# quantumgizmos/bp_osd

Hardware: AMD Instinct MI355X
Metric: syndromes decoded/sec (whole node) + logical error rate, HGP [[1922,50]] p=0.05 (higher is better)
Workload: dtype f64; 1 GPU; h1922_ms_cs7: [[1922,50]] HGP (31x31 circulant 1+x^2+x^5) hz 961x1922, min-sum BP variable scaling, max_iter=1922, osd_cs order 7, iid bit-flip q=0.05; per_gpu_batch=131072, global_batch=131072, bp_variant=0, pipelined_steps=2, hw_queues=4, batches=2 distinct seeded batches alternate over the timed steps

## Files before the change

### bp_osd_amd/_lib.py

```python
from __future__ import annotations

import ctypes as C
import os

_HERE = os.path.dirname(os.path.abspath(__file__))
LIB_PATH = os.environ.get("BPOSD_LIB") or os.path.join(_HERE, "libbposd_mi355x.so")

BPOSD_OK = 0
BPOSD_ERR_INVALID = -1
BPOSD_ERR_UNSUPPORTED = -2
BPOSD_ERR_HIP = -3
BPOSD_ERR_NO_DEVICE = -4

EXPORTED_SYMBOLS = (
    "bposd_device_count",
    "bposd_version",
    "bposd_create",
    "bposd_update_channel_probs",
    "bposd_decode_batch",
    "bposd_decode_batch_packed",
    "bposd_decode_batch_async",
    "bposd_decode_batch_packed_async",
    "bposd_decode_batch_device",
    "bposd_decode_batch_device_packed",
    "bposd_decode_batch_select",
    "bposd_decode_batch_select_device",
    "bposd_pack_rows_device",
    "bposd_pack_rows_device_lane",
    "bposd_synchronize",
    "bposd_num_lanes",
    "bposd_last_lane",
    "bposd_synchronize_lane",
    "bposd_lane_timing",
    "bposd_host_alloc",
    "bposd_host_free",
    "bposd_last_timing",
    "bposd_info",
    "bposd_posterior_llr",
    "bposd_set_bp_variant",
    "bposd_set_osd_variant",
    "bposd_last_osd_kernel",
    "bposd_mc_create",
    "bposd_mc_run",
    "bposd_mc_fetch",
    "bposd_mc_device_bytes",
    "bposd_mc_last_error",
    "bposd_mc_destroy",
    "bposd_last_error",
    "bposd_destroy",
)

DEBUG_SYMBOLS = (
    "bposd_layout_info",
    "bposd_bp_kernel_info",
    "bposd_debug_local_layout",
    "bposd_debug_class_layout",
    "bposd_debug_last_instance",
)


class BposdConfig(C.Structure):
    _fields_ = [
        ("device", C.c_int32),
        ("bp_method", C.c_int32),
        ("ms_scaling_factor", C.c_double),
        ("max_iter", C.c_int32),
        ("osd_method", C.c_int32),
        ("osd_order", C.c_int32),
        ("sort_tie_policy", C.c_int32),
        ("weight_fn", C.c_int32),
        ("schedule", C.c_int32),
        ("ps_clip", C.c_double),
        ("osd_e_bit_order", C.c_int32),
        ("ps_math_form", C.c_int32),
    ]


class BposdMcConfig(C.Structure):
    _fields_ = [
        ("device", C.c_int32),
        ("channel_update", C.c_int32),
        ("seed", C.c_uint64),
        ("capacity", C.c_int64),
    ]


MC_UPDATE = {None: 0, "x->z": 1, "z->x": 2}
MC_ITEMS = {"error_x": 0, "error_z": 1, "syndrome_x": 2, "syndrome_z": 3, "flags": 4, "syndrome_x_packed": 5, "syndrome_z_packed": 6}


_lib = None


def load():
    global _lib
    if _lib is not None:
        return _lib
    if not os.path.exists(LIB_PATH):
        raise RuntimeError(
            f"{LIB_PATH} not found: build it with `python -c 'import __graft_entry__ as g; g.build()'` "
            "(hipcc --offload-arch=gfx950).  bp_osd_amd has no CPU fallback."
        )
    os.environ.setdefault("GPU_MAX_HW_QUEUES", "8")
    lib = C.CDLL(LIB_PATH)
    vp = C.c_void_p
    lib.bposd_device_count.restype = C.c_int
    lib.bposd_version.restype = C.c_char_p
    lib.bposd_create.argtypes = [C.POINTER(BposdConfig), vp, vp, C.c_int32, C.c_int32, vp, C.POINTER(vp)]
    lib.bposd_create.restype = C.c_int
    lib.bposd_update_channel_probs.argtypes = [vp, vp]
    lib.bposd_update_channel_probs.restype = C.c_int
    lib.bposd_decode_batch.argtypes = [vp, vp, C.c_int64, vp, vp, vp, vp, vp, vp]
    lib.bposd_decode_batch.restype = C.c_int
    lib.bposd_decode_batch_packed.argtypes = [vp, vp, C.c_int64, vp, vp, vp, vp, vp]
    lib.bposd_decode_batch_packed.restype = C.c_int
    lib.bposd_decode_batch_async.argtypes = [vp, vp, C.c_int64, vp, vp, vp, vp, vp, vp]
    lib.bposd_decode_batch_async.restype = C.c_int
    lib.bposd_decode_batch_packed_async.argtypes = [vp, vp, C.c_int64, vp, vp, vp, vp, vp]
    lib.bposd_decode_batch_packed_async.restype = C.c_int
    lib.bposd_decode_batch_device.argtypes = [vp, vp, C.c_int64, vp, vp, vp, vp, vp, vp]
    lib.bposd_decode_batch_device.restype = C.c_int
    lib.bposd_decode_batch_device_packed.argtypes = [vp, vp, C.c_int64, vp, vp, vp, vp, vp]
    lib.bposd_decode_batch_device_packed.restype = C.c_int
    lib.bposd_decode_batch_select.argtypes = [vp, vp, C.c_int64, vp, vp, vp, vp, vp, vp, vp, vp]
    lib.bposd_decode_batch_select.restype = C.c_int
    lib.bposd_decode_batch_select_device.argtypes = [vp, vp, C.c_int64, vp, vp, vp, vp, vp, vp, vp, vp]
    lib.bposd_decode_batch_select_device.restype = C.c_int
    lib.bposd_pack_rows_device.argtypes = [vp, vp, C.c_int64, C.c_int32, vp]
    lib.bposd_pack_rows_device.restype = C.c_int
    lib.bposd_synchronize.argtypes = [vp]
    lib.bposd_synchronize.restype = C.c_int
    lib.bposd_num_lanes.argtypes = [vp]
    lib.bposd_num_lanes.restype = C.c_int
    lib.bposd_last_lane.argtypes = [vp]
    lib.bposd_last_lane.restype = C.c_int
    lib.bposd_synchronize_lane.argtypes = [vp, C.c_int32]
    lib.bposd_synchronize_lane.restype = C.c_int
    lib.bposd_lane_timing.argtypes = [vp, C.c_int32, C.POINTER(C.c_double), C.POINTER(C.c_double),
                                      C.POINTER(C.c_int64), C.POINTER(C.c_int64)]
    lib.bposd_lane_timing.restype = C.c_int
    lib.bposd_host_alloc.argtypes = [C.c_size_t]
    lib.bposd_host_alloc.restype = vp
    lib.bposd_host_free.argtypes = [vp]
    lib.bposd_host_free.restype = None
    lib.bposd_last_timing.argtypes = [vp, C.POINTER(C.c_double), C.POINTER(C.c_double),
                                      C.POINTER(C.c_int64), C.POINTER(C.c_int64)]
    lib.bposd_last_timing.restype = C.c_int
    lib.bposd_info.argtypes = [vp, C.POINTER(C.c_int32), C.POINTER(C.c_int32), C.POINTER(C.c_int32),
                               C.POINTER(C.c_int32)]
    lib.bposd_info.restype = C.c_int
    lib.bposd_layout_info.argtypes = [vp, C.POINTER(C.c_int64), C.POINTER(C.c_int64), C.POINTER(C.c_int64)]
    lib.bposd_layout_info.restype = C.c_int
    lib.bposd_pack_rows_device_lane.argtypes = [vp, C.c_int32, vp, C.c_int64, C.c_int32, vp]
    lib.bposd_pack_rows_device_lane.restype = C.c_int
    lib.bposd_posterior_llr.argtypes = [vp, vp, C.c_int64, vp, vp, vp, vp]
    lib.bposd_posterior_llr.restype = C.c_int
    lib.bposd_bp_kernel_info.argtypes = [vp, C.POINTER(C.c_int32), vp]
    lib.bposd_bp_kernel_info.restype = C.c_int
    lib.bposd_debug_local_layout.argtypes = [vp, vp, C.c_int32, C.c_int32, vp]
    lib.bposd_debug_local_layout.restype = C.c_int
    lib.bposd_debug_class_layout.argtypes = [vp, vp, C.c_int32, C.c_int32, vp, vp, vp, vp, vp, vp]
    lib.bposd_debug_class_layout.restype = C.c_int
    lib.bposd_debug_last_instance.argtypes = [vp, vp, vp]
    lib.bposd_debug_last_instance.restype = C.c_int
    lib.bposd_set_osd_variant.argtypes = [vp, C.c_int32]
    lib.bposd_set_osd_variant.restype = C.c_int
    lib.bposd_last_osd_kernel.argtypes = [vp]
    lib.bposd_last_osd_kernel.restype = C.c_int
    lib.bposd_set_bp_variant.argtypes = [vp, C.c_int32]
    lib.bposd_set_bp_variant.restype = C.c_int
    lib.bposd_last_error.argtypes = [vp]
    lib.bposd_last_error.restype = C.c_char_p
    lib.bposd_destroy.argtypes = [vp]
    lib.bposd_destroy.restype = None
    lib.bposd_mc_create.argtypes = [C.POINTER(BposdMcConfig), vp, vp, vp, vp, C.c_int32, vp, vp, C.c_int32, C.c_int32, vp, vp, C.c_int32,
                                    vp, vp, vp, vp, C.POINTER(vp)]
    lib.bposd_mc_create.restype = C.c_int
    lib.bposd_mc_run.argtypes = [vp, C.c_uint64, C.c_int64, C.POINTER(C.c_int64)]
    lib.bposd_mc_run.restype = C.c_int
    lib.bposd_mc_fetch.argtypes = [vp, C.c_int32, vp, C.c_size_t]
    lib.bposd_mc_fetch.restype = C.c_int
    lib.bposd_mc_device_bytes.argtypes = [vp]
    lib.bposd_mc_device_bytes.restype = C.c_int64
    lib.bposd_mc_last_error.argtypes = [vp]
    lib.bposd_mc_last_error.restype = C.c_char_p
    lib.bposd_mc_destroy.argtypes = [vp]
    lib.bposd_mc_destroy.restype = None
    _lib = lib
    return lib


def check_mc(lib, mc, rc):
    if rc == BPOSD_OK:
        return
    msg = lib.bposd_mc_last_error(mc)
    msg = msg.decode() if msg else f"error {rc}"
    if rc in (BPOSD_ERR_INVALID, BPOSD_ERR_UNSUPPORTED):
        raise ValueError(msg)
    raise RuntimeError(msg)


def check(lib, handle, rc):
    if rc == BPOSD_OK:
        return
    msg = lib.bposd_last_error(handle)
    msg = msg.decode() if msg else f"error {rc}"
    if rc in (BPOSD_ERR_INVALID, BPOSD_ERR_UNSUPPORTED):
        raise ValueError(msg)
    raise RuntimeError(msg)
```

### bp_osd_amd/csrc/bp_local_kernel.hip.h

```cpp
#pragma once
#include <hip/hip_runtime.h>
#include <stdint.h>

#include "bp_kernel.hip.h"

#ifndef BPOSD_BPL_SIGN_ON_MAG
#define BPOSD_BPL_SIGN_ON_MAG 0
#endif
namespace bposd {

struct BpLocalParams {
    int m, n;
    long long B;
    int max_iter;
    double ms_scaling;
    int osd_enabled;
    int mp;
    const uint8_t* __restrict__ synd;
    const double* __restrict__ llr0;
    const uint8_t* __restrict__ sel;
    const double* __restrict__ llr0_alt;
    const int* __restrict__ pos_chk;
    const int* __restrict__ pos_bit;
    const int* __restrict__ pos_alo;
    const int* __restrict__ pos_ahi;
    const int* __restrict__ pos_dl;
    const int* __restrict__ grp_dl;
    uint8_t* __restrict__ out_bp;
    uint8_t* __restrict__ out_osd0;
    uint8_t* __restrict__ out_osdw;
    uint8_t* __restrict__ out_conv;
    int* __restrict__ out_iters;
    double* __restrict__ out_llr;
    double* __restrict__ llr_ws;
    double* __restrict__ llr_tmp;
    int* __restrict__ osd_list;
    int* __restrict__ counters;
    unsigned long long* __restrict__ iter_total;
    int* __restrict__ tail_flag;
    int packed_io;
};

__host__ __device__ inline size_t bp_local_lds_bytes(int mp) {
    return ((size_t)4 * mp + 2) * 8 + (size_t)(mp / 32 + 2) * 4 + 8 * 4;
}

template <int DL>
__device__ __forceinline__ void bit_update(double l0, double R, double X, double Y, double& llr, double& oR, double& oX,
                                           double& oY) {
    const double c0 = DL == 0 ? R : (DL == 1 ? Y : X);
    const double c1 = DL == 0 ? X : (DL == 1 ? R : Y);
    const double c2 = DL == 0 ? Y : (DL == 1 ? X : R);
    const double pre0 = l0;
    const double pre1 = pre0 + c0;
    const double pre2 = pre1 + c1;
    llr = pre2 + c2;
    const double o2 = pre2;
    const double o1 = pre1 + c2;
    const double o0 = pre0 + (c2 + c1);
    oR = DL == 0 ? o0 : (DL == 1 ? o1 : o2);
    oX = DL == 0 ? o1 : (DL == 1 ? o2 : o0);
    oY = DL == 0 ? o2 : (DL == 1 ? o0 : o1);
}

__device__ __forceinline__ void bit_update_mixed(int dlv, double l0, double R, double X, double Y, double& llr, double& oR,
                                                 double& oX, double& oY) {
    const bool d0 = dlv == 0, d1 = dlv == 1;
    const double c0 = d0 ? R : (d1 ? Y : X);
    const double c1 = d0 ? X : (d1 ? R : Y);
    const double c2 = d0 ? Y : (d1 ? X : R);
    const double pre0 = l0;
    const double pre1 = pre0 + c0;
    const double pre2 = pre1 + c1;
    llr = pre2 + c2;
    const double o2 = pre2;
    const double o1 = pre1 + c2;
    const double o0 = pre0 + (c2 + c1);
    oR = d0 ? o0 : (d1 ? o1 : o2);
    oX = d0 ? o1 : (d1 ? o2 : o0);
    oY = d0 ? o2 : (d1 ? o0 : o1);
}

__device__ __forceinline__ int bpl_table_load(const int* base, unsigned int lane_off, unsigned int const_off) {
    asm volatile("" : "+v"(lane_off));
    return *(const int*)((const char*)base + (lane_off + const_off));
}

static_assert(__is_trivially_copyable(BpLocalParams) && alignof(BpLocalParams) <= 8, "BpLocalParams is copied into the kernarg segment as it is");
typedef const __attribute__((address_space(4))) BpLocalParams* bpl_args_ptr;
__device__ __forceinline__ bpl_args_ptr bpl_args() {
    bpl_args_ptr a = (bpl_args_ptr)__builtin_amdgcn_kernarg_segment_ptr();
    asm volatile("" : "+s"(a));
    return a;
}

template <int CPT, int MPT, int MINW, bool EARLY, bool UPRIOR, bool PACKED = false>
__global__ __launch_bounds__(MPT / CPT, MINW) void bp_local_kernel(const BpLocalParams P) {
    extern __shared__ __attribute__((aligned(16))) unsigned char smem[];
    const int m = P.m, n = P.n;
#ifdef BPOSD_DEBUG
    if (blockIdx.x == 0 && threadIdx.x == 0 && (bpl_args()->m != P.m || bpl_args()->counters != P.counters)) __builtin_trap();
#endif
    constexpr int NT = MPT / CPT;
    constexpr int MP = MPT;
    const int tid = threadIdx.x;
    const int lane = tid & 63;
    const int wave = __builtin_amdgcn_readfirstlane(tid >> 6);
    constexpr int NB = 2 * CPT;

    double* msg_plain = reinterpret_cast<double*>(smem);
    msg_ptr msg = (msg_ptr)msg_plain;
    unsigned int* diffw = reinterpret_cast<unsigned int*>(msg_plain + (size_t)4 * MP + 2);
    int* sh = reinterpret_cast<int*>(diffw + (MP / 32 + 2));
    const unsigned int diffw_base = (unsigned int)(uintptr_t)(__attribute__((address_space(3))) unsigned char*)diffw;

    typedef __attribute__((address_space(3))) unsigned char* lds_bytes;
    const unsigned int msg_base = (unsigned int)(uintptr_t)(lds_bytes)smem;
    unsigned int alo[NB], ahi[NB];
    int dl[NB];
    unsigned int dlpack = 0u;
    double l0[UPRIOR ? 1 : NB];
    if (UPRIOR) {
        const double v = bpl_args()->llr0[0];
        l0[0] = __hiloint2double(__builtin_amdgcn_readfirstlane(__double2hiint(v)), __builtin_amdgcn_readfirstlane(__double2loint(v)));
    }
#define BPL_L0(r) l0[UPRIOR ? 0 : (r)]
#define BPL_AT(a) ((msg_ptr)(uintptr_t)(a))
#define BPL_BIT(r) bpl_table_load(bpl_args()->pos_bit, (unsigned int)tid * 4u, (unsigned int)((((r) & 1) * MP + ((r) >> 1) * NT) * 4))
#pragma unroll
    for (int j = 0; j < CPT; ++j) {
        const int p = tid + j * NT;
#pragma unroll
        for (int b = 0; b < 2; ++b) {
            const int r = 2 * j + b;
            if (!UPRIOR) {
                const int bit = BPL_BIT(r);
                l0[r] = bit >= 0 ? bpl_args()->llr0[bit] : 1.0;
            }
            alo[r] = msg_base + 8u * (unsigned int)bpl_args()->pos_alo[b * MP + p];
            ahi[r] = msg_base + 8u * (unsigned int)bpl_args()->pos_ahi[b * MP + p];
            dl[r] = __builtin_amdgcn_readfirstlane(bpl_args()->grp_dl[b * (MP >> 6) + (p >> 6)]);
            dlpack |= (unsigned int)bpl_args()->pos_dl[b * MP + p] << (2 * r);
        }
    }

    const int want_llr_s = __builtin_amdgcn_readfirstlane(bpl_args()->out_llr != nullptr ? 1 : 0);
    auto want_llr = [&]() -> bool {
        int w = want_llr_s;
        asm volatile("" : "+s"(w));
        return w != 0;
    };
    for (;;) {
        if (tid == 0) {
            int zero = 0;
            asm volatile("" : "+v"(zero));
            sh[0] = zero;
            sh[1] = zero;
            sh[2] = atomicAdd(&bpl_args()->counters[0], 1);
        }
        __syncthreads();
        const long long s = __builtin_amdgcn_readfirstlane(sh[2]);
        if (s >= P.B) {
            if (s == P.B && tid == 0 && bpl_args()->tail_flag) *(volatile int*)bpl_args()->tail_flag = 1;
            break;
        }

        bool sbit[CPT];
#pragma unroll
        for (int j = 0; j < CPT; ++j) {
            const int c = bpl_table_load(bpl_args()->pos_chk, (unsigned int)tid * 4u, (unsigned int)(j * NT * 4));
            sbit[j] = (c >= 0) ? (PACKED ? bp_synd_bit(bpl_args()->synd, 1, s, m, c) : ((bpl_args()->synd[(size_t)s * m + c] & 1) != 0)) : false;
            const unsigned long long bal = __ballot(sbit[j]);
            if (lane == 0) {
                const int w0 = ((wave << 6) + j * NT) >> 5;
                diffw[w0] = (unsigned int)bal;
                diffw[w0 + 1] = (unsigned int)(bal >> 32);
                if (bal) sh[0] = 1;
            }
        }
        if (!UPRIOR && bpl_args()->sel) {
#pragma unroll
            for (int j = 0; j < CPT; ++j)
#pragma unroll
                for (int b = 0; b < 2; ++b) {
                    const int i = BPL_BIT(2 * j + b);
                    if (i >= 0) l0[2 * j + b] = bpl_args()->sel[(size_t)s * n + i] ? bpl_args()->llr0_alt[i] : bpl_args()->llr0[i];
                }
        }
        double loc[NB];
#define BPL_LLRT (bpl_args()->llr_tmp + (size_t)blockIdx.x * n)
        unsigned int decmask = 0u;
#pragma unroll
        for (int r = 0; r < NB; ++r) {
            double lp = BPL_L0(r);
            if (UPRIOR) asm volatile("" : "+s"(lp));
            loc[r] = lp;
            *BPL_AT(alo[r]) = lp;
            *BPL_AT(ahi[r]) = lp;
        }
        if (want_llr()) {
#pragma unroll
            for (int r = 0; r < NB; ++r) {
                const int i = BPL_BIT(r);
                double lp = BPL_L0(r);
                if (UPRIOR) asm volatile("" : "+s"(lp));
                if (i >= 0) BPL_LLRT[i] = lp;
            }
        }
        __syncthreads();

        int it_done = 0;
        bool conv = (sh[0] == 0);
        if (!conv) {
#pragma clang loop unroll(disable)
            for (int it = 1;; ++it) {
                const int fi = it & 1;
                {
                    unsigned long long mis = 0ull;
#pragma unroll
                    for (int j = 0; j < CPT; ++j)
                        mis |= *(const volatile __attribute__((address_space(3))) unsigned long long*)(uintptr_t)(
                            diffw_base + (unsigned int)(((wave << 6) + j * NT) >> 3));
                    if (lane == 0 && mis) sh[fi] = 1;
                }
                if (it > P.max_iter) {
                    __syncthreads();
                    conv = (sh[fi] == 0);
                    it_done = P.max_iter;
                    break;
                }
                const unsigned long long alpha_u = alpha_bits_for_iteration(P.ms_scaling, it);
                const int alpha_lo = (int)(unsigned int)alpha_u, alpha_hi = (int)(unsigned int)(alpha_u >> 32), nalpha_hi = alpha_hi ^ (int)0x80000000;
                double vl[EARLY ? CPT : 1][4];
                if (EARLY) {
#pragma unroll
                    for (int j = 0; j < CPT; ++j)
#pragma unroll
                        for (int k = 0; k < 4; ++k) vl[j][k] = msg[(tid + j * NT) + k * MP];
                }
#pragma unroll
                for (int j = 0; j < CPT; ++j) {
                    msg_ptr mc = msg + (tid + j * NT);
                    double v[6];
#pragma unroll
                    for (int k = 0; k < 4; ++k) v[k] = EARLY ? vl[j][k] : mc[k * MP];
                    v[4] = loc[2 * j];
                    v[5] = loc[2 * j + 1];
                    double pre[6], suf[6];
                    pre[0] = __DBL_MAX__;
#pragma unroll
                    for (int k = 1; k < 6; ++k) pre[k] = min_abs(pre[k - 1], v[k - 1]);
                    suf[5] = __DBL_MAX__;
#pragma unroll
                    for (int k = 4; k >= 0; --k) suf[k] = min_abs(suf[k + 1], v[k + 1]);
#if BPOSD_BPL_SIGN_ON_MAG
                    unsigned long long negm[6];
                    unsigned long long parm = __ballot(sbit[j]);
#pragma unroll
                    for (int k = 0; k < 6; ++k) {
                        negm[k] = __ballot(v[k] <= 0.0);
                        parm ^= negm[k];
                    }
                    const double alpha_d = __hiloint2double(alpha_hi, alpha_lo);
#pragma unroll
                    for (int k = 0; k < 6; ++k) {
                        const double mag = (k == 0) ? suf[0] : (k == 5 ? pre[5] : min_pos(pre[k], suf[k]));
                        const unsigned long long selm = parm ^ negm[k];
                        int mh = __double2hiint(mag);
                        asm("v_cndmask_b32_e64 %0, %1, -%1, %2" : "=v"(mh) : "v"(mh), "s"(selm));
                        const double o = __hiloint2double(mh, __double2loint(mag)) * alpha_d;
                        if (k < 4) mc[k * MP] = o;
                        else loc[2 * j + (k - 4)] = o;
                    }
#else
                    bool neg[6];
                    bool par = sbit[j];
#pragma unroll
                    for (int k = 0; k < 6; ++k) {
                        neg[k] = (v[k] <= 0.0);
                        par ^= neg[k];
                    }
#pragma unroll
                    for (int k = 0; k < 6; ++k) {
                        const double mag = (k == 0) ? suf[0] : (k == 5 ? pre[5] : min_pos(pre[k], suf[k]));
                        const double sa = __hiloint2double((par ^ neg[k]) ? nalpha_hi : alpha_hi, alpha_lo);
                        const double o = mag * sa;
                        if (k < 4) mc[k * MP] = o;
                        else loc[2 * j + (k - 4)] = o;
                    }
#endif
                }
                __syncthreads();
                if (sh[fi] == 0) {
                    conv = true;
                    it_done = it - 1;
                    break;
                }
                if (tid == 0) sh[fi ^ 1] = 0;
                const bool keep_llr = (it == P.max_iter) || want_llr();
#ifndef BPOSD_BPL_BATCH
#define BPOSD_BPL_BATCH 2
#endif
                constexpr int BATCH = (MINW >= 8 && NB > 2) ? BPOSD_BPL_BATCH : NB;
                double X[NB], Y[NB];
#pragma unroll
                for (int r = 0; r < NB; ++r) {
                    if (r % BATCH == 0) {
#pragma unroll
                        for (int q = r; q < r + BATCH; ++q) {
                            X[q] = *BPL_AT(alo[q]);
                            Y[q] = *BPL_AT(ahi[q]);
                        }
                    }
                    double oR, oX, oY, t;
                    if (dl[r] == 0) bit_update<0>(BPL_L0(r), loc[r], X[r], Y[r], t, oR, oX, oY);
                    else if (dl[r] == 1) bit_update<1>(BPL_L0(r), loc[r], X[r], Y[r], t, oR, oX, oY);
                    else if (dl[r] == 2) bit_update<2>(BPL_L0(r), loc[r], X[r], Y[r], t, oR, oX, oY);
                    else bit_update_mixed((int)((dlpack >> (2 * r)) & 3u), BPL_L0(r), loc[r], X[r], Y[r], t, oR, oX, oY);
                    if (keep_llr) {
                        const int bi = BPL_BIT(r);
                        if (bi >= 0) BPL_LLRT[bi] = t;
                    }
                    loc[r] = oR;
                    *BPL_AT(alo[r]) = oX;
                    *BPL_AT(ahi[r]) = oY;
                    const unsigned int dnew = (t <= 0.0) ? 1u : 0u;
                    if (dnew != ((decmask >> r) & 1u)) {
                        decmask ^= 1u << r;
                        unsigned int pa = alo[r], pb = ahi[r];
                        asm volatile("" : "+v"(pa), "+v"(pb));
                        const int ca = (int)((pa - msg_base) >> 3) & (MP - 1), cb = (int)((pb - msg_base) >> 3) & (MP - 1);
                        const int co = tid + (r >> 1) * NT;
                        atomicXor(&diffw[ca >> 5], 1u << (ca & 31));
                        atomicXor(&diffw[cb >> 5], 1u << (cb & 31));
                        atomicXor(&diffw[co >> 5], 1u << (co & 31));
                    }
                }
                __syncthreads();
            }
        }

        const bool to_osd = (!conv) && bpl_args()->osd_enabled;
        if (tid == 0) {
            if (to_osd) {
                const int slot = atomicAdd(&bpl_args()->counters[1], 1);
                bpl_args()->osd_list[slot] = (int)s;
                sh[3] = slot;
            }
            if (bpl_args()->out_conv) bpl_args()->out_conv[s] = conv ? 1 : 0;
            if (bpl_args()->out_iters) bpl_args()->out_iters[s] = it_done;
            if (it_done) atomicAdd(bpl_args()->iter_total, (unsigned long long)it_done);
        }
        __syncthreads();
        const int slot = to_osd ? sh[3] : 0;
        constexpr bool packed = PACKED;
        if (packed)
            bp_store_packed_rows<NB>((unsigned int*)smem, tid, NT, n, s, to_osd, (unsigned long long*)bpl_args()->out_bp,
                                     (unsigned long long*)bpl_args()->out_osd0, (unsigned long long*)bpl_args()->out_osdw,
                                     [&](int r) { return BPL_BIT(r); }, [&](int r) { return ((decmask >> r) & 1u) != 0u; });
#pragma unroll
        for (int r = 0; r < NB; ++r) {
            const int i = BPL_BIT(r);
            if (i >= 0) {
                const size_t o = (size_t)s * n + i;
                const uint8_t b = (uint8_t)((decmask >> r) & 1u);
                if (!packed) {
                    if (bpl_args()->out_bp) bpl_args()->out_bp[o] = b;
                    if (!to_osd) {
                        bpl_args()->out_osdw[o] = b;
                        if (bpl_args()->out_osd0) bpl_args()->out_osd0[o] = b;
                    }
                }
                if (to_osd) bpl_args()->llr_ws[(size_t)slot * n + i] = BPL_LLRT[i];
                if (want_llr()) bpl_args()->out_llr[o] = BPL_LLRT[i];
            }
        }
        __syncthreads();
    }
}

#undef BPL_L0
#undef BPL_AT
#undef BPL_BIT
#undef BPL_LLRT

}
```

### bp_osd_amd/csrc/bposd_capi.hip

```cpp
#include "../../include/bposd_mi355x.h"

#include <hip/hip_runtime.h>

#include <algorithm>
#include <cmath>
#include <cstdarg>
#include <cstdio>
#include <cstdlib>
#include <climits>
#include <cstring>
#include <string>
#include <tuple>
#include <functional>
#include <map>
#include <chrono>
#include <mutex>
#include <thread>
#include <vector>

#include "internal.h"
#include <array>
#include <vector>
#include <algorithm>
#include "local_layout.h"
// ... 251 lines not shown
}

int build_tables(bposd_handle* h, int DC, int DV, int MP, int NT, int VPT) {
    const int m = h->m, n = h->n, NP = NT * VPT;
    std::vector<int> bit_of_pos;
    choose_bit_layout(h, MP, NT, VPT, bit_of_pos);
    std::vector<int> pos_of_bit(n, -1);
    for (int p = 0; p < NP; ++p)
        if (bit_of_pos[p] >= 0) pos_of_bit[bit_of_pos[p]] = p;
    std::vector<int> chk_deg(m), var_deg(NP, 0);
    std::vector<int> var_pos((size_t)DV * NP, 0);
    for (int c = 0; c < m; ++c) {
        chk_deg[c] = h->rp[c + 1] - h->rp[c];
        for (int e = h->rp[c]; e < h->rp[c + 1]; ++e) {
            const int k = e - h->rp[c];
            const int p = pos_of_bit[h->ci[e]];
            const int d = var_deg[p]++;
            var_pos[(size_t)d * NP + p] = k * MP + c;
        }
    }
    auto up = [&](int** dst, const std::vector<int>& v) -> int {
        if (*dst) { (void)hipFree(*dst); *dst = nullptr; }
        HIP_TRY(h, hipMalloc((void**)dst, sizeof(int) * std::max<size_t>(v.size(), 1)));
        HIP_TRY(h, hipMemcpy(*dst, v.data(), sizeof(int) * v.size(), hipMemcpyHostToDevice));
        return 0;
    };
    int rc;
    if ((rc = up(&h->d_chk_deg, chk_deg))) return rc;
    if ((rc = up(&h->d_var_deg, var_deg))) return rc;
    if ((rc = up(&h->d_var_pos, var_pos))) return rc;
    if ((rc = up(&h->d_pos_bit, bit_of_pos))) return rc;
    h->tab_dc = DC;
    h->tab_dv = DV;
    h->tab_mp = MP;
    h->tab_np = NP;
    return 0;
}
int build_tables_local(bposd_handle* h) {
    using namespace local_layout;
    h->local_ok = false;
    const int m = h->m, n = h->n;
    if (!(h->regular && h->dc_max == 6 && h->dv_max == 3 && n == 2 * m)) return 0;
    const int MP = m <= 1024 ? 1024 : 2048;
    if (m > MP) return 0;
    Graph g;
    Layout best;
    if (!local_layout_host(h->rp, h->ci, m, n, MP, g, best)) return 0;
    if (getenv("BPOSD_DEBUG_OCC"))
        fprintf(stderr, "[bposd] local-edge layout: bit pass %lld read cycles (floor %d) + %lld write cycles (floor %d), %d mixed pairs, %d uniform positions\n",
                best.passes, 4 * (MP / 32), best.wcycles, 6 * 4 * (MP / 64), best.mixed, best.nfull);
    h->local_passes = best.passes;
    h->local_wcycles = best.wcycles;

    const int G = MP / 64;
    const std::vector<int>&owner = best.owner, &load = best.load, &pos_of = best.pos_of, &pos_chk = best.pos_chk;
    std::vector<int> grp_dl(2 * (size_t)G, 0);
    for (int gq = 0; gq < G; ++gq)
        for (int b = 0; b < 2; ++b) {
            int code = -1;
            for (int p = 64 * gq; p < 64 * gq + 64; ++p) {
                const int c = pos_chk[p];
                if (c < 0) continue;
                const int d = g.rank_of(load[2 * c + b], c);
                code = (code < 0 || code == d) ? d : 3;
            }
            grp_dl[(size_t)b * G + gq] = code < 0 ? 0 : code;
        }
    auto slot_of = [&](int c, int i) {
        int k = 0;
        for (int e = h->rp[c]; e < h->rp[c + 1]; ++e) {
            const int j = h->ci[e];
            if (owner[j] == c) continue;
            if (j == i) return k * MP + pos_of[c];
            ++k;
        }
        return -1;
    };
    std::vector<int> pos_bit(2 * (size_t)MP, -1), pos_alo(2 * (size_t)MP, 0), pos_ahi(2 * (size_t)MP, 0), pos_dl(2 * (size_t)MP, 0);
    for (int p = 0; p < MP; ++p)
        for (int b = 0; b < 2; ++b) {
            pos_alo[(size_t)b * MP + p] = (2 * b) * MP + p;
            pos_ahi[(size_t)b * MP + p] = (2 * b + 1) * MP + p;
        }
    for (int c = 0; c < m; ++c) {
        const int p = pos_of[c];
        for (int b = 0; b < 2; ++b) {
            const int i = load[2 * c + b];
            int o[2];
            g.others(i, c, o);
            const int sx = slot_of(o[0], i), sy = slot_of(o[1], i);
            if (sx < 0 || sy < 0) return 0;
            pos_dl[(size_t)b * MP + p] = g.rank_of(i, c);
            pos_bit[(size_t)b * MP + p] = i;
            pos_alo[(size_t)b * MP + p] = sx;
            pos_ahi[(size_t)b * MP + p] = sy;
        }
    }
    auto up = [&](int** dst, const std::vector<int>& v) -> int {
        if (*dst) { (void)hipFree(*dst); *dst = nullptr; }
        HIP_TRY(h, hipMalloc((void**)dst, sizeof(int) * std::max<size_t>(v.size(), 1)));
        HIP_TRY(h, hipMemcpy(*dst, v.data(), sizeof(int) * v.size(), hipMemcpyHostToDevice));
        return 0;
    };
    int rc;
    if ((rc = up(&h->d_lpos_chk, pos_chk))) return rc;
    if ((rc = up(&h->d_lpos_bit, pos_bit))) return rc;
    if ((rc = up(&h->d_lpos_alo, pos_alo))) return rc;
    if ((rc = up(&h->d_lpos_ahi, pos_ahi))) return rc;
    if ((rc = up(&h->d_lgrp_dl, grp_dl))) return rc;
    if ((rc = up(&h->d_lpos_dl, pos_dl))) return rc;
    h->local_mp = MP;
    h->local_ok = true;
    return 0;
}
struct ClassShape { int dclo, dc, dvlo, dvhi; };
const ClassShape kClassShapes[] = {{7, 7, 3, 4}, {6, 6, 3, 3}, {4, 4, 2, 2}, {8, 8, 4, 4}, {3, 4, 1, 2}};
constexpr int kClassVPT = 2;

const ClassShape* class_shape_for(const std::vector<int>& rp, const std::vector<int>& ci, int m, int n) {
    int clo = 1 << 30, chi = 0, lo = 1 << 30, hi = 0;
// ... 1214 lines not shown
}

int bposd_lane_timing(bposd_handle* h, int32_t lane, double* bp_ms, double* osd_ms, int64_t* bp_iterations,
                      int64_t* osd_invocations) {
    if (!h) return BPOSD_ERR_INVALID;
    if (lane < 0 || lane >= BPOSD_LANES) return fail(h, BPOSD_ERR_INVALID, "lane %d out of range", lane);
    if (!h->have_timing) return fail(h, BPOSD_ERR_INVALID, "no decode call has been made on this handle");
    DeviceGuard dev_guard(h->device);
    HIP_TRY(h, dev_guard.err);
    HIP_TRY(h, hipStreamSynchronize(h->lanes[lane].stream));
    return record_timing(h, &h->lane_rec[lane], 1, bp_ms, osd_ms, bp_iterations, osd_invocations);
}

int bposd_debug_local_layout(const int32_t* indptr, const int32_t* indices, int32_t m, int32_t n, int64_t* out) {
    if (!indptr || !indices || !out || n != 2 * m) return BPOSD_ERR_INVALID;
    std::vector<int> rp(indptr, indptr + m + 1), ci(indices, indices + indptr[m]);
    const int MP = m <= 1024 ? 1024 : 2048;
    if (m > MP) return BPOSD_ERR_UNSUPPORTED;
    for (int c = 0; c < m; ++c)
        if (rp[c + 1] - rp[c] != 6) return BPOSD_ERR_UNSUPPORTED;
    std::vector<int> deg(n, 0);
    for (int e : ci) {
        if (e < 0 || e >= n) return BPOSD_ERR_INVALID;
        deg[e]++;
    }
    for (int i = 0; i < n; ++i)
        if (deg[i] != 3) return BPOSD_ERR_UNSUPPORTED;
    local_layout::Graph g;
    local_layout::Layout best;
    if (!local_layout_host(rp, ci, m, n, MP, g, best)) return BPOSD_ERR_UNSUPPORTED;
    int mixed = 0;
    for (int gq = 0; gq < MP / 64; ++gq)
        for (int b = 0; b < 2; ++b) {
            int code = -1;
            for (int p = 64 * gq; p < 64 * gq + 64; ++p) {
                const int c = best.pos_chk[p];
                if (c < 0) continue;
                const int d = g.rank_of(best.load[2 * c + b], c);
                code = (code < 0 || code == d) ? d : 3;
            }
            mixed += code == 3;
        }
    out[0] = best.passes; out[1] = 4 * (MP / 32); out[2] = best.nfull; out[3] = mixed; out[4] = MP;
    out[14] = best.wcycles; out[15] = 6 * 4 * (MP / 64);
    for (int k = 0; k < 9; ++k) out[5 + k] = 0;
    for (int c = 0; c < m; ++c) {
        int a = g.rank_of(best.load[2 * c], c), b = g.rank_of(best.load[2 * c + 1], c);
        if (a > b) std::swap(a, b);
        out[5 + a * 3 + b]++;
    }
    return BPOSD_OK;
}

int bposd_debug_class_layout(const int32_t* indptr, const int32_t* indices, int32_t m, int32_t n, int32_t* pos_chk, int32_t* pos_bit,
                             int32_t* bit_slot, int32_t* grp_deg, int32_t* grp_cdeg, int64_t* info) {
    if (!indptr || !indices || !info || m < 1 || n < 1) return BPOSD_ERR_INVALID;
    std::vector<int> rp(indptr, indptr + m + 1), ci(indices, indices + indptr[m]);
    for (int e : ci)
        if (e < 0 || e >= n) return BPOSD_ERR_INVALID;
    const ClassShape* shp = class_shape_for(rp, ci, m, n);
    if (!shp || m > 1024) return BPOSD_ERR_UNSUPPORTED;
    class_layout::Tables T;
    bool ok = false;
    for (int mp : {256, 512, 1024}) {
        if (m > mp) continue;
        if (class_layout::build(rp, ci, m, n, shp->dclo, shp->dc, shp->dvlo, shp->dvhi, kClassVPT, mp, mp, class_layout_iters(), T)) { ok = true; break; }
    }
    if (!ok) return BPOSD_ERR_UNSUPPORTED;
    info[0] = shp->dc; info[1] = shp->dvlo; info[2] = shp->dvhi; info[3] = kClassVPT; info[4] = T.MP; info[5] = T.NT;
    info[6] = T.read_cycles; info[7] = T.read_floor; info[8] = T.write_cycles; info[9] = T.write_floor; info[10] = shp->dclo;
    if (pos_chk) std::copy(T.pos_chk.begin(), T.pos_chk.end(), pos_chk);
    if (pos_bit) std::copy(T.pos_bit.begin(), T.pos_bit.end(), pos_bit);
    if (bit_slot) std::copy(T.bit_slot.begin(), T.bit_slot.end(), bit_slot);
    if (grp_deg) std::copy(T.grp_deg.begin(), T.grp_deg.end(), grp_deg);
    if (grp_cdeg) std::copy(T.grp_cdeg.begin(), T.grp_cdeg.end(), grp_cdeg);
    return BPOSD_OK;
}

void* bposd_host_alloc(size_t bytes) {
    void* p = nullptr;
    if (bytes == 0 || hipHostMalloc(&p, bytes, hipHostMallocDefault) != hipSuccess) return nullptr;
    return p;
}

void bposd_host_free(void* p) {
    if (p) (void)hipHostFree(p);
}

}
```

### bp_osd_amd/csrc/local_layout.h

```cpp
#pragma once
#include <algorithm>
#include <cmath>
#include <cstdio>
#include <cstdlib>
#include <functional>
#include <thread>
#include <vector>

namespace local_layout {

struct Layout {
    std::vector<int> owner;
    std::vector<int> load;
    std::vector<int> pos_of;
    std::vector<int> pos_chk;
    int nfull = 0;
    double cost = 1e30;
    long long passes = 0;
    long long wcycles = 0;
    int mixed = 0;
};

struct Graph {
    int m, n, MP;
    std::vector<int> cols;
    int rank_of(int i, int c) const { return cols[3 * (size_t)i] == c ? 0 : (cols[3 * (size_t)i + 1] == c ? 1 : 2); }
    void others(int i, int c, int* o) const {
        const int d = rank_of(i, c);
        o[0] = cols[3 * (size_t)i + (d + 1) % 3];
        o[1] = cols[3 * (size_t)i + (d + 2) % 3];
    }
};

struct LdsCost {
    int read_cycles = 0, write_cycles = 0, mixed = 0;
};

struct BitPassModel {
    const Graph& g;
    Layout& L;
    std::vector<int> tgt;
    std::vector<std::vector<int>> users;
    BitPassModel(const Graph& g_, Layout& L_) : g(g_), L(L_), tgt(4 * (size_t)g_.m), users(g_.m) {
        for (int c = 0; c < g.m; ++c)
            for (int b = 0; b < 2; ++b) {
                int o[2];
                g.others(L.load[2 * c + b], c, o);
                for (int s = 0; s < 2; ++s) {
                    tgt[4 * (size_t)c + 2 * b + s] = o[s];
                    users[o[s]].push_back(4 * c + 2 * b + s);
                }
            }
    }
    int column(int p, int bs) const {
        const int c = L.pos_chk[p];
        return c < 0 ? p : L.pos_of[tgt[4 * (size_t)c + bs]];
    }
    void group_cost(int gq, int bs, int& rd, int& wr, int& pairs) const {
        int c32[2][32] = {{0}}, c16[4][16] = {{0}};
        rd = 0; pairs = 0;
        int wsum = 0;
        int mx32[2] = {0, 0}, mx16[4] = {0, 0, 0, 0};
        for (int l = 0; l < 64; ++l) {
            const int col = column(64 * gq + l, bs);
            int& a = c32[l >> 5][col & 31];
            pairs += a;
            if (++a > mx32[l >> 5]) mx32[l >> 5] = a;
            int& w = c16[l >> 4][col & 15];
            pairs += w;
            if (++w > mx16[l >> 4]) mx16[l >> 4] = w;
        }
        rd = mx32[0] + mx32[1];
        wsum = mx16[0] + mx16[1] + mx16[2] + mx16[3];
// ... 177 lines not shown
        bool closed = false;
        int cur = c0;
        for (int depth = 0; depth < 6 && !closed; ++depth) {
            const int b = L.load[2 * cur + rnd(2)];
            if (std::find(path_bit.begin(), path_bit.end(), b) != path_bit.end()) break;
            int o[2];
            g.others(b, cur, o);
            int nxt = -1;
            if (depth > 0 && (o[0] == c0 || o[1] == c0)) nxt = c0;
            else nxt = o[rnd(2)];
            if (nxt != c0 && std::find(path_chk.begin(), path_chk.end(), nxt) != path_chk.end()) break;
            path_bit.push_back(b);
            if (nxt == c0) closed = true;
            else { path_chk.push_back(nxt); cur = nxt; }
        }
        if (!closed || path_bit.size() < 2) continue;
        const size_t len = path_bit.size();
        int before[8], after_[8];
        for (size_t t = 0; t < len; ++t) before[t] = key(path_chk[t]);
        for (size_t t = 0; t < len; ++t) {
            const int from = path_chk[t], to = path_chk[(t + 1) % len];
            replace_bit(to, path_bit[(t + 1) % len], -2 - (int)t);
            (void)from;
        }
        for (size_t t = 0; t < len; ++t) {
            const int to = path_chk[(t + 1) % len];
            replace_bit(to, -2 - (int)t, path_bit[t]);
            L.owner[path_bit[t]] = to;
        }
        for (size_t t = 0; t < len; ++t) { after_[t] = key(path_chk[t]); cnt[before[t]]--; }
        for (size_t t = 0; t < len; ++t) cnt[after_[t]]++;
        const int F2 = groups_needed(cnt), S2 = slack();
        if (F2 < F || (F2 == F && (S2 < S || (sideways && (S2 == S || rnd(8) == 0))))) { F = F2; S = S2; continue; }
        for (size_t t = 0; t < len; ++t) { cnt[after_[t]]--; }
        for (size_t t = 0; t < len; ++t) { cnt[before[t]]++; }
        for (size_t t = 0; t < len; ++t) {
            const int to = path_chk[(t + 1) % len];
            replace_bit(to, path_bit[t], -2 - (int)t);
        }
        for (size_t t = 0; t < len; ++t) {
            const int to = path_chk[(t + 1) % len];
            replace_bit(to, -2 - (int)t, path_bit[(t + 1) % len]);
            L.owner[path_bit[(t + 1) % len]] = to;
        }
    }
    if (getenv("BPOSD_DEBUG_OCC")) {
        fprintf(stderr, "[bposd] class rebalancing: groups needed %d (available %d), classes", F, G);
        for (int k = 0; k < 9; ++k) fprintf(stderr, " %d", cnt[k]);
        fprintf(stderr, "\n");
    }
    return F <= G;
}

}

inline bool local_layout_host(const std::vector<int>& rp, const std::vector<int>& ci, int m, int n, int MP,
                              local_layout::Graph& g, local_layout::Layout& best) {
    using namespace local_layout;
    g.m = m; g.n = n; g.MP = MP;
    g.cols.assign(3 * (size_t)n, 0);
    {
        std::vector<int> fill(n, 0);
        for (int c = 0; c < m; ++c)
            for (int e = rp[c]; e < rp[c + 1]; ++e) {
                const int i = ci[e];
                g.cols[3 * (size_t)i + fill[i]++] = c;
            }
    }
    const std::vector<int>& cols = g.cols;
    std::vector<Layout> cands;
    {
        Layout L;
        L.owner.assign(n, -1);
        L.load.assign(2 * (size_t)m, -1);
        auto cnt = [&](int c) { return (L.load[2 * c] >= 0) + (L.load[2 * c + 1] >= 0); };
        auto put = [&](int c, int i) { (L.load[2 * c] < 0 ? L.load[2 * c] : L.load[2 * c + 1]) = i; L.owner[i] = c; };
        auto drop = [&](int c, int i) { if (L.load[2 * c] == i) L.load[2 * c] = -1; else L.load[2 * c + 1] = -1; };
        std::vector<int> seen(m, -1);
        std::function<bool(int, int)> place = [&](int i, int stamp) -> bool {
            for (int d = 0; d < 3; ++d) {
                const int c = cols[3 * (size_t)i + d];
                if (seen[c] == stamp) continue;
                seen[c] = stamp;
                if (cnt(c) < 2) { put(c, i); return true; }
                for (int s2 = 0; s2 < 2; ++s2) {
                    const int j = L.load[2 * c + s2];
                    drop(c, j);
                    L.owner[j] = -1;
                    if (place(j, stamp)) { put(c, i); return true; }
                    L.load[2 * c + s2] = j;
                    L.owner[j] = c;
                }
            }
            return false;
        };
        for (int i = 0; i < n; ++i)
            if (!place(i, i)) return false;
        for (int c = 0; c < m; ++c)
            if (cnt(c) != 2) return false;
        cands.push_back(L);
    }
    bool two_block = true;
    for (int c = 0; c < m && two_block; ++c) {
        int lo = 0;
        for (int e = rp[c]; e < rp[c + 1]; ++e) lo += ci[e] < n / 2;
        two_block = (lo == 3);
    }
    if (two_block) {
        std::vector<int> own2(n), slot(2 * (size_t)m), seen2(m);
        for (int p1 = 0; p1 < 3; ++p1)
// ... 12 lines not shown
                        if (j < 0 || aug(j, stamp, blk)) { slot[2 * c + blk] = i; own2[i] = c; return true; }
                    }
                    return false;
                };
                int stamp = 0;
                for (int i = 0; i < n; ++i) (void)aug(i, ++stamp, i < n / 2 ? 0 : 1);
                pref_only = false;
                bool ok = true;
                for (int i = 0; i < n && ok; ++i)
                    if (own2[i] < 0) ok = aug(i, ++stamp, i < n / 2 ? 0 : 1);
                for (int c = 0; c < m && ok; ++c) ok = slot[2 * c] >= 0 && slot[2 * c + 1] >= 0;
                if (!ok) continue;
                Layout L;
                L.owner = own2;
                L.load = slot;
                cands.push_back(L);
            }
    }
    {
        const size_t n0 = cands.size();
        for (size_t k = 0; k < n0; ++k)
            for (int sideways = 0; sideways < 2; ++sideways) {
                Layout R = cands[k];
                if (rebalance_classes(g, R, MP / 64, 100000, sideways != 0)) { cands.push_back(R); break; }
            }
    }
    {
        double mixw = 5.0;
        if (const char* e = getenv("BPOSD_MIXW")) mixw = atof(e);
        auto total = [&](const Layout& L) { return L.cost - 5.0 * L.mixed + mixw * L.mixed; };
        std::vector<std::pair<double, size_t>> rank;
        for (size_t k = 0; k < cands.size(); ++k) {
            class_sorted(g, cands[k]);
            search(g, cands[k], true, 0);
            rank.push_back({total(cands[k]), k});
        }
        std::sort(rank.begin(), rank.end());
        const size_t nfinish = std::min(rank.size(), getenv("BPOSD_LAYOUT_ALL") ? rank.size() : (size_t)3);
        const int iters = getenv("BPOSD_LAYOUT_ITERS") ? atoi(getenv("BPOSD_LAYOUT_ITERS")) : 400000;
        std::vector<Layout> fin(nfinish);
        std::vector<std::thread> th;
        for (size_t q = 0; q < nfinish; ++q) {
            fin[q] = cands[rank[q].second];
            th.emplace_back([&g, &fin, q, iters]() { search(g, fin[q], true, iters); });
        }
        for (auto& t : th) t.join();
        for (size_t q = 0; q < nfinish; ++q) {
            if (getenv("BPOSD_DEBUG_OCC"))
                fprintf(stderr, "[bposd] candidate %zu: %lld read + %lld write cycles, %d mixed pairs\n", rank[q].second, fin[q].passes,
                        fin[q].wcycles, fin[q].mixed);
            if (q == 0 || total(fin[q]) < total(best)) best = fin[q];
        }
    }
    return true;
}
```

### include/bposd_mi355x_debug.h

```cpp
#ifndef BPOSD_MI355X_DEBUG_H
#define BPOSD_MI355X_DEBUG_H

#include "bposd_mi355x.h"

#ifdef __cplusplus
extern "C" {
#endif
#pragma GCC visibility push(default)

int bposd_layout_info(bposd_handle *h, int64_t *natural_cycles, int64_t *chosen_cycles, int64_t *ideal_cycles);

#define BPOSD_BP_KERNEL_LDS 0
#define BPOSD_BP_KERNEL_LOCAL 1
#define BPOSD_BP_KERNEL_CLASS 2
#define BPOSD_BP_KERNEL_LARGE 3
#define BPOSD_BP_KERNEL_SERIAL 4
#define BPOSD_BP_KERNEL_ANYDEG 5
int bposd_bp_kernel_info(bposd_handle *h, int32_t *kernel, int64_t *lds_model);

int bposd_debug_last_instance(bposd_handle *h, int32_t bp[6], int32_t osd[6]);

int bposd_debug_local_layout(const int32_t *csr_indptr, const int32_t *csr_indices, int32_t m, int32_t n, int64_t *out);

int bposd_debug_class_layout(const int32_t *csr_indptr, const int32_t *csr_indices, int32_t m, int32_t n, int32_t *pos_chk,
                             int32_t *pos_bit, int32_t *bit_slot, int32_t *grp_deg, int32_t *grp_cdeg, int64_t *info);

#pragma GCC visibility pop
#ifdef __cplusplus
}
#endif
#endif
```

Measured before the change: 5.483 million syndromes/s.

## Pair same-key check groups into waves and specialise BP bit pass per wave key

The host layout now permutes 64-check groups so that the two groups handled by each wave share the same degree-rank key. The BP local kernel then takes a wave-uniform key and dispatches to a compile-time-specialised iteration loop, removing per-bit runtime branches on dl. It also splits off the LLR-keeping final iteration into a separate loop instance. The cost is more kernel code (larger instruction footprint, possible register pressure), and waves with mixed keys still fall back to a generic per-group switch.

```diff
diff --git a/bp_osd_amd/_lib.py b/bp_osd_amd/_lib.py
--- a/bp_osd_amd/_lib.py
+++ b/bp_osd_amd/_lib.py
@@ -54,6 +54,7 @@
     "bposd_layout_info",
     "bposd_bp_kernel_info",
     "bposd_debug_local_layout",
+    "bposd_debug_local_keys",
     "bposd_debug_class_layout",
     "bposd_debug_last_instance",
 )
@@ -159,6 +160,8 @@
     lib.bposd_bp_kernel_info.restype = C.c_int
     lib.bposd_debug_local_layout.argtypes = [vp, vp, C.c_int32, C.c_int32, vp]
     lib.bposd_debug_local_layout.restype = C.c_int
+    lib.bposd_debug_local_keys.argtypes = [vp, vp, C.c_int32, C.c_int32, vp, vp, vp]
+    lib.bposd_debug_local_keys.restype = C.c_int
     lib.bposd_debug_class_layout.argtypes = [vp, vp, C.c_int32, C.c_int32, vp, vp, vp, vp, vp, vp]
     lib.bposd_debug_class_layout.restype = C.c_int
     lib.bposd_debug_last_instance.argtypes = [vp, vp, vp]
diff --git a/bp_osd_amd/csrc/bp_local_kernel.hip.h b/bp_osd_amd/csrc/bp_local_kernel.hip.h
--- a/bp_osd_amd/csrc/bp_local_kernel.hip.h
+++ b/bp_osd_amd/csrc/bp_local_kernel.hip.h
@@ -3,6 +3,7 @@
 #include <stdint.h>
 
 #include "bp_kernel.hip.h"
+#include "local_keys.h"
 
 #ifndef BPOSD_BPL_SIGN_ON_MAG
 #define BPOSD_BPL_SIGN_ON_MAG 0
@@ -94,6 +95,15 @@
     return a;
 }
 
+template <int V>
+struct bpl_int {
+    static constexpr int value = V;
+};
+
+__host__ __device__ constexpr bool bpl_specialised(int cpt, int mpt, int minw, bool early) {
+    return !early && ((cpt == 1 && mpt == 1024 && minw == 8) || (cpt == 2 && mpt == 1024 && (minw == 8 || minw == 6)) || (cpt == 2 && mpt == 2048 && minw == 4));
+}
+
 template <int CPT, int MPT, int MINW, bool EARLY, bool UPRIOR, bool PACKED = false>
 __global__ __launch_bounds__(MPT / CPT, MINW) void bp_local_kernel(const BpLocalParams P) {
     extern __shared__ __attribute__((aligned(16))) unsigned char smem[];
@@ -144,6 +154,14 @@
         }
     }
 
+    int gkey[CPT];
+#pragma unroll
+    for (int j = 0; j < CPT; ++j) gkey[j] = bposd_local_keys::group_key(dl[2 * j], dl[2 * j + 1]);
+    int wkey = gkey[0];
+#pragma unroll
+    for (int j = 1; j < CPT; ++j) wkey = (gkey[j] == wkey) ? wkey : -1;
+    constexpr bool SPEC = bpl_specialised(CPT, MPT, MINW, EARLY);
+
     const int want_llr_s = __builtin_amdgcn_readfirstlane(bpl_args()->out_llr != nullptr ? 1 : 0);
     auto want_llr = [&]() -> bool {
         int w = want_llr_s;
@@ -210,10 +228,14 @@
         __syncthreads();
 
         int it_done = 0;
-        bool conv = (sh[0] == 0);
-        if (!conv) {
+        int conv = __builtin_amdgcn_readfirstlane(sh[0]) == 0 ? 1 : 0;
+        auto iterate = [&](auto key_c, auto llr_c, const int it0) __attribute__((always_inline)) -> int {
+            constexpr int KEY = decltype(key_c)::value;
+            constexpr bool LLR = decltype(llr_c)::value;
+            const int max_iter = bpl_args()->max_iter;
 #pragma clang loop unroll(disable)
-            for (int it = 1;; ++it) {
+            for (int it = it0; LLR || it < max_iter; ++it) {
+                asm volatile("; bpl_body key=%0 llr=%1" ::"n"(KEY), "n"((int)LLR));
                 const int fi = it & 1;
                 {
                     unsigned long long mis = 0ull;
@@ -223,11 +245,11 @@
                             diffw_base + (unsigned int)(((wave << 6) + j * NT) >> 3));
                     if (lane == 0 && mis) sh[fi] = 1;
                 }
-                if (it > P.max_iter) {
+                if (LLR && it > max_iter) {
                     __syncthreads();
-                    conv = (sh[fi] == 0);
-                    it_done = P.max_iter;
-                    break;
+                    conv = __builtin_amdgcn_readfirstlane(sh[fi]) == 0 ? 1 : 0;
+                    it_done = max_iter;
+                    return 1;
                 }
                 const unsigned long long alpha_u = alpha_bits_for_iteration(P.ms_scaling, it);
                 const int alpha_lo = (int)(unsigned int)alpha_u, alpha_hi = (int)(unsigned int)(alpha_u >> 32), nalpha_hi = alpha_hi ^ (int)0x80000000;
@@ -291,33 +313,24 @@
 #endif
                 }
                 __syncthreads();
-                if (sh[fi] == 0) {
-                    conv = true;
+                if (__builtin_amdgcn_readfirstlane(sh[fi]) == 0) {
+                    conv = 1;
                     it_done = it - 1;
-                    break;
+                    return 1;
                 }
                 if (tid == 0) sh[fi ^ 1] = 0;
-                const bool keep_llr = (it == P.max_iter) || want_llr();
 #ifndef BPOSD_BPL_BATCH
 #define BPOSD_BPL_BATCH 2
 #endif
                 constexpr int BATCH = (MINW >= 8 && NB > 2) ? BPOSD_BPL_BATCH : NB;
+                static_assert(BATCH % 2 == 0 && NB % BATCH == 0, "the bit pass loads the messages of whole groups");
                 double X[NB], Y[NB];
-#pragma unroll
-                for (int r = 0; r < NB; ++r) {
-                    if (r % BATCH == 0) {
-#pragma unroll
-                        for (int q = r; q < r + BATCH; ++q) {
-                            X[q] = *BPL_AT(alo[q]);
-                            Y[q] = *BPL_AT(ahi[q]);
-                        }
-                    }
+                auto bit_step = [&](const int r, auto dl_c) __attribute__((always_inline)) {
+                    constexpr int DL = decltype(dl_c)::value;
                     double oR, oX, oY, t;
-                    if (dl[r] == 0) bit_update<0>(BPL_L0(r), loc[r], X[r], Y[r], t, oR, oX, oY);
-                    else if (dl[r] == 1) bit_update<1>(BPL_L0(r), loc[r], X[r], Y[r], t, oR, oX, oY);
-                    else if (dl[r] == 2) bit_update<2>(BPL_L0(r), loc[r], X[r], Y[r], t, oR, oX, oY);
-                    else bit_update_mixed((int)((dlpack >> (2 * r)) & 3u), BPL_L0(r), loc[r], X[r], Y[r], t, oR, oX, oY);
-                    if (keep_llr) {
+                    if constexpr (DL == 3) bit_update_mixed((int)((dlpack >> (2 * r)) & 3u), BPL_L0(r), loc[r], X[r], Y[r], t, oR, oX, oY);
+                    else bit_update<DL>(BPL_L0(r), loc[r], X[r], Y[r], t, oR, oX, oY);
+                    if (LLR) {
                         const int bi = BPL_BIT(r);
                         if (bi >= 0) BPL_LLRT[bi] = t;
                     }
@@ -335,9 +348,61 @@
                         atomicXor(&diffw[cb >> 5], 1u << (cb & 31));
                         atomicXor(&diffw[co >> 5], 1u << (co & 31));
                     }
+                };
+                auto group_step = [&](const int j, auto gk_c) __attribute__((always_inline)) {
+                    constexpr int GK = decltype(gk_c)::value;
+                    bit_step(2 * j, bpl_int<bposd_local_keys::key_dl(GK, 0)>{});
+                    bit_step(2 * j + 1, bpl_int<bposd_local_keys::key_dl(GK, 1)>{});
+                };
+#pragma unroll
+                for (int j = 0; j < CPT; ++j) {
+                    if ((2 * j) % BATCH == 0) {
+#pragma unroll
+                        for (int q = 2 * j; q < 2 * j + BATCH; ++q) {
+                            X[q] = *BPL_AT(alo[q]);
+                            Y[q] = *BPL_AT(ahi[q]);
+                        }
+                    }
+                    if constexpr (KEY >= 0) group_step(j, bpl_int<KEY>{});
+                    else {
+                        switch (gkey[j]) {
+                            case 0: group_step(j, bpl_int<0>{}); break;
+                            case 1: group_step(j, bpl_int<1>{}); break;
+                            case 2: group_step(j, bpl_int<2>{}); break;
+                            case 5: group_step(j, bpl_int<5>{}); break;
+                            case 6: group_step(j, bpl_int<6>{}); break;
+                            case 10: group_step(j, bpl_int<10>{}); break;
+                            default: group_step(j, bpl_int<bposd_local_keys::kMixedKey>{}); break;
+                        }
+                    }
                 }
                 __syncthreads();
             }
+            return 0;
+        };
+        if (!conv) {
+            int done = 0;
+            int it_llr = 1;
+            if (!want_llr()) {
+                int wk = wkey;
+                asm volatile("" : "+s"(wk));
+                if constexpr (SPEC) {
+                    switch (wk) {
+                        case 0: done = iterate(bpl_int<0>{}, bpl_int<0>{}, 1); break;
+                        case 1: done = iterate(bpl_int<1>{}, bpl_int<0>{}, 1); break;
+                        case 2: done = iterate(bpl_int<2>{}, bpl_int<0>{}, 1); break;
+                        case 5: done = iterate(bpl_int<5>{}, bpl_int<0>{}, 1); break;
+                        case 6: done = iterate(bpl_int<6>{}, bpl_int<0>{}, 1); break;
+                        case 10: done = iterate(bpl_int<10>{}, bpl_int<0>{}, 1); break;
+                        case bposd_local_keys::kMixedKey: done = iterate(bpl_int<bposd_local_keys::kMixedKey>{}, bpl_int<0>{}, 1); break;
+                        default: done = iterate(bpl_int<-1>{}, bpl_int<0>{}, 1); break;
+                    }
+                } else done = iterate(bpl_int<-1>{}, bpl_int<0>{}, 1);
+                asm volatile("" : "+s"(done));
+                it_llr = bpl_args()->max_iter;
+                it_llr = it_llr > 1 ? it_llr : 1;
+            }
+            if (!done) iterate(bpl_int<-1>{}, bpl_int<1>{}, it_llr);
         }
 
         const bool to_osd = (!conv) && bpl_args()->osd_enabled;
diff --git a/bp_osd_amd/csrc/bposd_capi.hip b/bp_osd_amd/csrc/bposd_capi.hip
--- a/bp_osd_amd/csrc/bposd_capi.hip
+++ b/bp_osd_amd/csrc/bposd_capi.hip
@@ -327,20 +327,8 @@
     h->local_passes = best.passes;
     h->local_wcycles = best.wcycles;
 
-    const int G = MP / 64;
     const std::vector<int>&owner = best.owner, &load = best.load, &pos_of = best.pos_of, &pos_chk = best.pos_chk;
-    std::vector<int> grp_dl(2 * (size_t)G, 0);
-    for (int gq = 0; gq < G; ++gq)
-        for (int b = 0; b < 2; ++b) {
-            int code = -1;
-            for (int p = 64 * gq; p < 64 * gq + 64; ++p) {
-                const int c = pos_chk[p];
-                if (c < 0) continue;
-                const int d = g.rank_of(load[2 * c + b], c);
-                code = (code < 0 || code == d) ? d : 3;
-            }
-            grp_dl[(size_t)b * G + gq] = code < 0 ? 0 : code;
-        }
+    const std::vector<int> grp_dl = group_dl_table(g, best);
     auto slot_of = [&](int c, int i) {
         int k = 0;
         for (int e = h->rp[c]; e < h->rp[c + 1]; ++e) {
@@ -1661,6 +1649,35 @@
     return BPOSD_OK;
 }
 
+int bposd_debug_local_keys(const int32_t* indptr, const int32_t* indices, int32_t m, int32_t n, int32_t* group_key, int32_t* pos_chk, int64_t* info) {
+    if (!indptr || !indices || !group_key || !pos_chk || !info || n != 2 * m) return BPOSD_ERR_INVALID;
+    std::vector<int> rp(indptr, indptr + m + 1), ci(indices, indices + indptr[m]);
+    const int MP = m <= 1024 ? 1024 : 2048;
+    if (m > MP) return BPOSD_ERR_UNSUPPORTED;
+    for (int c = 0; c < m; ++c)
+        if (rp[c + 1] - rp[c] != 6) return BPOSD_ERR_UNSUPPORTED;
+    std::vector<int> deg(n, 0);
+    for (int e : ci) {
+        if (e < 0 || e >= n) return BPOSD_ERR_INVALID;
+        deg[e]++;
+    }
+    for (int i = 0; i < n; ++i)
+        if (deg[i] != 3) return BPOSD_ERR_UNSUPPORTED;
+    local_layout::Graph g;
+    local_layout::Layout best;
+    if (!local_layout_host(rp, ci, m, n, MP, g, best, false)) return BPOSD_ERR_UNSUPPORTED;
+    local_layout::LdsCost t = local_layout::lds_cost(g, best);
+    info[0] = t.read_cycles; info[1] = t.write_cycles; info[2] = t.mixed;
+    if (local_layout::pair_groups(g, best) < 0) return BPOSD_ERR_UNSUPPORTED;
+    t = local_layout::lds_cost(g, best);
+    info[3] = t.read_cycles; info[4] = t.write_cycles; info[5] = t.mixed;
+    info[6] = MP; info[7] = best.generic_waves;
+    const std::vector<int> keys = local_layout::group_keys(g, best);
+    for (int gq = 0; gq < MP / 64; ++gq) group_key[gq] = keys[gq];
+    for (int p = 0; p < MP; ++p) pos_chk[p] = best.pos_chk[p];
+    return BPOSD_OK;
+}
+
 int bposd_debug_class_layout(const int32_t* indptr, const int32_t* indices, int32_t m, int32_t n, int32_t* pos_chk, int32_t* pos_bit,
                              int32_t* bit_slot, int32_t* grp_deg, int32_t* grp_cdeg, int64_t* info) {
     if (!indptr || !indices || !info || m < 1 || n < 1) return BPOSD_ERR_INVALID;
diff --git a/bp_osd_amd/csrc/local_keys.h b/bp_osd_amd/csrc/local_keys.h
--- /dev/null
+++ b/bp_osd_amd/csrc/local_keys.h
@@ -0,0 +1,12 @@
+#pragma once
+
+namespace bposd_local_keys {
+
+constexpr int kMixedKey = 15;
+constexpr int kNumKeys = 7;
+constexpr int kKeys[kNumKeys] = {0, 1, 2, 5, 6, 10, 15};
+
+constexpr int group_key(int dl0, int dl1) { return (dl0 >= 0 && dl0 <= dl1 && dl1 < 3) ? 4 * dl0 + dl1 : kMixedKey; }
+constexpr int key_dl(int key, int slot) { return key == kMixedKey ? 3 : (slot == 0 ? key / 4 : key % 4); }
+
+}
diff --git a/bp_osd_amd/csrc/local_layout.h b/bp_osd_amd/csrc/local_layout.h
--- a/bp_osd_amd/csrc/local_layout.h
+++ b/bp_osd_amd/csrc/local_layout.h
@@ -6,6 +6,8 @@
 #include <functional>
 #include <thread>
 #include <vector>
+
+#include "local_keys.h"
 
 namespace local_layout {
 
@@ -19,6 +21,7 @@
     long long passes = 0;
     long long wcycles = 0;
     int mixed = 0;
+    int generic_waves = 0;
 };
 
 struct Graph {
@@ -302,10 +305,83 @@
     return F <= G;
 }
 
+inline int group_code(const Graph& g, const Layout& L, int gq, int b) {
+    int code = -1;
+    for (int p = 64 * gq; p < 64 * gq + 64; ++p) {
+        const int c = L.pos_chk[p];
+        if (c < 0) continue;
+        const int d = g.rank_of(L.load[2 * c + b], c);
+        code = (code < 0 || code == d) ? d : 3;
+    }
+    return code;
+}
+
+inline std::vector<int> group_dl_table(const Graph& g, const Layout& L) {
+    const int G = g.MP / 64;
+    std::vector<int> t(2 * (size_t)G, 0);
+    for (int gq = 0; gq < G; ++gq)
+        for (int b = 0; b < 2; ++b) {
+            int code = group_code(g, L, gq, b);
+            if (code < 0) code = group_code(g, L, (gq + G / 2) % G, b);
+            t[(size_t)b * G + gq] = code < 0 ? 0 : code;
+        }
+    return t;
+}
+
+inline std::vector<int> group_keys(const Graph& g, const Layout& L) {
+    const int G = g.MP / 64;
+    const std::vector<int> t = group_dl_table(g, L);
+    std::vector<int> k(G);
+    for (int gq = 0; gq < G; ++gq) k[gq] = bposd_local_keys::group_key(t[gq], t[(size_t)G + gq]);
+    return k;
+}
+
+inline int pair_groups(const Graph& g, Layout& L) {
+    const int G = g.MP / 64, W = G / 2;
+    std::vector<int> key(G);
+    for (int gq = 0; gq < G; ++gq) {
+        const int c0 = group_code(g, L, gq, 0), c1 = group_code(g, L, gq, 1);
+        key[gq] = c0 < 0 ? -1 : bposd_local_keys::group_key(c0, c1);
+    }
+    std::vector<std::pair<int, int>> pairs;
+    std::vector<int> singles, empties;
+    std::vector<char> used(G, 0);
+    for (int gq = 0; gq < G; ++gq) {
+        if (used[gq]) continue;
+        if (key[gq] < 0) { empties.push_back(gq); used[gq] = 1; continue; }
+        int mate = -1;
+        for (int q = gq + 1; q < G && mate < 0; ++q)
+            if (!used[q] && key[q] == key[gq]) mate = q;
+        used[gq] = 1;
+        if (mate < 0) { singles.push_back(gq); continue; }
+        used[mate] = 1;
+        pairs.push_back({gq, mate});
+    }
+    int generic = 0;
+    size_t e = 0, s1 = 0;
+    for (; s1 < singles.size() && e < empties.size(); ++s1, ++e) pairs.push_back({std::min(singles[s1], empties[e]), std::max(singles[s1], empties[e])});
+    for (; s1 + 1 < singles.size(); s1 += 2, ++generic) pairs.push_back({singles[s1], singles[s1 + 1]});
+    for (; e + 1 < empties.size(); e += 2) pairs.push_back({empties[e], empties[e + 1]});
+    if ((int)pairs.size() != W) return -1;
+    std::sort(pairs.begin(), pairs.end());
+    std::vector<int> new_of(G);
+    for (int w = 0; w < W; ++w) { new_of[pairs[w].first] = w; new_of[pairs[w].second] = w + W; }
+    std::vector<int> pos_chk(g.MP, -1);
+    for (int p = 0; p < g.MP; ++p) {
+        const int c = L.pos_chk[p];
+        const int q = 64 * new_of[p >> 6] + (p & 63);
+        pos_chk[q] = c;
+        if (c >= 0) L.pos_of[c] = q;
+    }
+    L.pos_chk = pos_chk;
+    L.generic_waves = generic;
+    return generic;
+}
+
 }
 
 inline bool local_layout_host(const std::vector<int>& rp, const std::vector<int>& ci, int m, int n, int MP,
-                              local_layout::Graph& g, local_layout::Layout& best) {
+                              local_layout::Graph& g, local_layout::Layout& best, bool pair = true) {
     using namespace local_layout;
     g.m = m; g.n = n; g.MP = MP;
     g.cols.assign(3 * (size_t)n, 0);
@@ -424,5 +500,13 @@
             if (q == 0 || total(fin[q]) < total(best)) best = fin[q];
         }
     }
+    if (pair) {
+        if (pair_groups(g, best) < 0) return false;
+        const LdsCost t = lds_cost(g, best);
+        best.passes = t.read_cycles;
+        best.wcycles = t.write_cycles;
+        best.mixed = t.mixed;
+        if (getenv("BPOSD_DEBUG_OCC")) fprintf(stderr, "[bposd] wave pairing: %d generic wave(s) of %d\n", best.generic_waves, MP / 128);
+    }
     return true;
 }
diff --git a/include/bposd_mi355x_debug.h b/include/bposd_mi355x_debug.h
--- a/include/bposd_mi355x_debug.h
+++ b/include/bposd_mi355x_debug.h
@@ -22,6 +22,9 @@
 
 int bposd_debug_local_layout(const int32_t *csr_indptr, const int32_t *csr_indices, int32_t m, int32_t n, int64_t *out);
 
+int bposd_debug_local_keys(const int32_t *csr_indptr, const int32_t *csr_indices, int32_t m, int32_t n, int32_t *group_key,
+                           int32_t *pos_chk, int64_t *info);
+
 int bposd_debug_class_layout(const int32_t *csr_indptr, const int32_t *csr_indices, int32_t m, int32_t n, int32_t *pos_chk,
                              int32_t *pos_bit, int32_t *bit_slot, int32_t *grp_deg, int32_t *grp_cdeg, int64_t *info);
 
```

Measured after the change: 5.606 million syndromes/s (median of 6 runs). 1.02x the previous value.
